# Lingeng56/conformer-pytorch-lightning

Measured on AMD Instinct MI355X. Metric: encoder frames/sec (80-d fbank, T=1000), whole job, higher is better.
Workload: dtype bf16

## Files before the change

conformer-pytorch-lightning_amd/csrc/encoder.cpp:

```cpp
#include <math.h>

#include <stdlib.h>

#include "cfm_common.h"

namespace {

inline const void* eoff(const void* p, int64_t elems, int dt) { return (const char*)p + elems * cfm_elt_size(dt); }

struct Ctx {
    const cfm_layer_io* io;
    int M, D, FF, act_dt, w_dt;
    bool split;
    cfm_stream_t st;
};

int gemm(const Ctx& c, const void* A, int a_dt, int64_t lda, const void* W, const void* Wlo, const float* bias, void* C, int c_dt,
         int64_t ldc, int M, int N, int K, int act, const float* res, float alpha, const uint8_t* row_mask) {
    cfm_gemm_desc d = {};
    d.A = A; d.W = W; d.W_lo = c.split ? Wlo : nullptr; d.bias = bias; d.residual = res; d.row_mask = row_mask; d.C = C;
    d.lda = lda; d.ldc = ldc; d.ldr = ldc; d.M = M; d.N = N; d.K = K;
    d.a_dtype = a_dt; d.w_dtype = c.w_dt; d.c_dtype = c_dt; d.act = act; d.alpha = alpha;
    if (c.split && !Wlo) return cfm_fail(CFM_ERR_ARG, "encoder layer: split mode needs the *_lo weight planes");
    return cfm_gemm(&d, c.st);
// ... 65 lines not shown
    auto after_tail = [&]() -> int {
        if (!io->after_out) return CFM_OK;
        return cfm_layernorm(x_out, io->after_g, io->after_b, io->after_out, CFM_F32, nullptr, nullptr, nullptr, 0, nullptr, eps, M, D, stream);
    };
    CFM_CHECK_ARG(!io->macaron_done || chains, "encoder layer: macaron_done needs the chain path");
    bool ring_written = false;
    static const int ffsplit_rows = getenv("CFM_FFSPLIT_MAX_ROWS") ? atoi(getenv("CFM_FFSPLIT_MAX_ROWS")) : CFM_FFSPLIT_MAX_ROWS;
    const bool ffsplit = chains && s->psum && M <= ffsplit_rows && cfm_ffn_split_supported(D, FF) && s->psum_splits >= FF / 256 &&
                         !io->macaron_done && !io->next_w && w->pw2_w && io->ktaps == 15;
    auto split_desc = [&](int mode) {
        cfm_ffn_split_desc f = {};
        f.M = M; f.D = D; f.mode = mode; f.w_dtype = c.w_dt; f.eps = eps;
        return f;
    };
    const bool pair = chains && s->psum && s->psum_splits >= 3 && M <= CFM_PAIR_MAX_ROWS && cfm_rowchain_pair_supported(D, FF) && !io->macaron_done && !io->next_w;
    if (pair) {
        cfm_rowchain_desc m = {};
        m.x = x_in; m.ln_g = w->ln_ffm_g; m.ln_b = w->ln_ffm_b; m.w1f = w->ffm_w1f; m.w2n = w->ffm_w2n; m.b1 = w->ffm_b1; m.b2 = w->ffm_b2;
        m.psum_out = s->psum; m.M = M; m.D = D; m.FF = FF; m.w_dtype = c.w_dt; m.alpha = 0.5f; m.eps = eps;
        CFM_TRY(cfm_rowchain(&m, stream));
        cfm_rowchain_desc q = {};
        q.x = x_in; q.psum_in = s->psum; q.psum_b2 = w->ffm_b2; q.psum_alpha = 0.5f; q.out_f32 = x_out; q.ln_g = w->ln_mha_g; q.ln_b = w->ln_mha_b;
        q.tail_w = w->qkv_wf; q.tail_b = w->qkv_b; q.tail_out = s->qkv; q.tail_N = 3 * D; q.M = M; q.D = D; q.FF = FF; q.w_dtype = c.w_dt; q.alpha = 1.0f; q.eps = eps;
        q.tail_pair = 1;
        CFM_TRY(cfm_rowchain(&q, stream));
    } else if (ffsplit) {
        cfm_ffn_split_desc f = split_desc(2);
        f.x = x_in; f.ln_g = w->ln_ffm_g; f.ln_b = w->ln_ffm_b; f.w1 = w->ffm_w1f; f.b1 = w->ffm_b1; f.N1 = FF; f.act = CFM_ACT_SILU; f.w2 = w->ffm_w2n;
        f.psum_out = s->psum;
        CFM_TRY(cfm_ffn_split(&f, stream));
        cfm_ffn_split_desc q = split_desc(1);
        q.x = x_in; q.psum = s->psum; q.psum_b2 = w->ffm_b2; q.psum_splits = FF / 256; q.psum_alpha = 0.5f; q.rows_out = x_out;
        q.ln_g = w->ln_mha_g; q.ln_b = w->ln_mha_b; q.w1 = w->qkv_wf; q.b1 = w->qkv_b; q.N1 = 3 * D; q.act = CFM_ACT_NONE; q.out16 = s->qkv; q.ldo = 3 * D;
        ring_written = ring && dk % 4 == 0;
        if (ring_written) { q.kv_ring = io->kv_ring; q.ring_offsets = io->stream_offset; q.ring_T = io->ring_T; q.ring_H = H; q.ring_Tq = io->T; }
        CFM_TRY(cfm_ffn_split(&q, stream));
    } else if (chains && !io->macaron_done && !pair) {
        cfm_rowchain_desc m = {};
        m.x = x_in; m.ln_g = w->ln_ffm_g; m.ln_b = w->ln_ffm_b; m.w1f = w->ffm_w1f; m.w2n = w->ffm_w2n; m.b1 = w->ffm_b1; m.b2 = w->ffm_b2;
        m.ln2_g = w->ln_mha_g; m.ln2_b = w->ln_mha_b; m.out_f32 = x_out; m.tail_w = w->qkv_wf; m.tail_b = w->qkv_b; m.tail_out = s->qkv;
        m.M = M; m.D = D; m.FF = FF; m.tail_N = 3 * D; m.tail_glu = 0; m.w_dtype = c.w_dt; m.alpha = 0.5f; m.eps = eps;
        CFM_TRY(cfm_rowchain(&m, stream));
    }
    const bool fused_ffn = !chains && !c.split && w->ffm_w1f && w->ffm_w2f && w->ff_w1f && w->ff_w2f && (D == 144 || D == 256) &&
                           FF % 32 == 0 && FF <= 2048;

    if (chains) {
    } else if (fused_ffn) {
        CFM_TRY(ffn_fused(c, x_in, w->ln_ffm_g, w->ln_ffm_b, w->ffm_w1f, w->ffm_w2f, w->ffm_b1, w->ffm_b2, nullptr, nullptr,
                          w->ln_mha_g, w->ln_mha_b, x_out, s->xn));
    } else {
        if (!xn_ready) CFM_TRY(cfm_layernorm(x_in, w->ln_ffm_g, w->ln_ffm_b, nullptr, 0, nullptr, nullptr, s->xn, adt, nullptr, eps, M, D, stream));
        CFM_TRY(gemm(c, s->xn, adt, D, w->ffm_w1, w->ffm_w1_lo, w->ffm_b1, s->hid, adt, FF, M, FF, D, CFM_ACT_SILU, nullptr, 0.f, nullptr));
        CFM_TRY(gemm(c, s->hid, adt, FF, w->ffm_w2, w->ffm_w2_lo, w->ffm_b2, x_out, CFM_F32, D, M, D, FF, CFM_ACT_NONE, x_in, 0.5f, nullptr));
        CFM_TRY(cfm_layernorm(x_out, w->ln_mha_g, w->ln_mha_b, nullptr, 0, nullptr, nullptr, s->xn, adt, nullptr, eps, M, D, stream));
// ... 24 lines not shown
        a.k_sb = a.v_sb = sb; a.k_sh = a.v_sh = dk; a.k_st = a.v_st = stt;
    }
    if (has_pos) {
        const int64_t pld = io->pos_proj ? io->pos_proj_ld : D;
        a.p = io->pos_proj ? io->pos_proj : s->pos; a.p_dtype = adt; a.p_sb = io->pos_shared ? 0 : (int64_t)P * pld; a.p_st = P == 1 ? 0 : pld;
        a.bias_u = w->bias_u; a.bias_v = w->bias_v;
    }
    a.mask = io->attn_mask; a.m_sb = io->am_sb; a.m_sq = io->am_sq;
    a.out = s->ctx; a.out_dtype = adt;
    a.B = io->B; a.H = H; a.Tq = io->T; a.Tk = Tk; a.dk = dk;
    a.mma_dtype = c.w_dt; a.split = c.split ? 1 : 0;
    a.scale = 1.0f / sqrtf((float)dk);
    CFM_TRY(cfm_attention(&a, stream));
    if (chains) {
        cfm_rowchain_desc ci = {};
        ci.head_a = s->ctx; ci.head_w = w->out_wf; ci.head_b = w->out_b; ci.head_res = x_out; ci.ln_g = w->ln_conv_g; ci.ln_b = w->ln_conv_b;
        ci.ln_mask = io->pad_valid; ci.out_f32 = x_out; ci.tail_w = w->pw1_wf; ci.tail_b = w->pw1_b; ci.tail_out = s->glu;
        ci.M = M; ci.D = D; ci.FF = FF; ci.tail_N = 2 * D; ci.tail_glu = 1; ci.w_dtype = c.w_dt; ci.alpha = 1.0f; ci.eps = eps;
        if (pair) { ci.tail_pair = 1; ci.out_f32 = s->psum + (int64_t)2 * M * D; }
        const bool cin = cin_merge_flag() != 0 && !pair && !ffsplit && io->next_w && io->next_x_out && D == 256 && FF == 2048 && io->ktaps == 15 && !io->causal_conv &&
                         !io->after_out;
        if (!cin) CFM_TRY(cfm_rowchain(&ci, stream));
        const bool dw_fused = io->ktaps == 15 && !io->causal_conv && cfm_rowchain_dw_supported(D);
        const bool pair_dw = pair && io->ktaps == 15 && !io->causal_conv;
        if (io->causal_conv) {
            CFM_TRY(cfm_dwconv_causal_bn_silu(s->glu, adt, io->conv_cache, w->dw_w, w->dw_b, w->bn_scale, w->bn_shift, s->dw, adt, io->B, io->T, D, io->ktaps, stream));
            if (io->conv_cache) CFM_TRY(cfm_conv_cache_update(s->glu, adt, io->conv_cache, io->B, io->T, D, io->ktaps, stream));
        } else if (!dw_fused && !pair_dw)
            CFM_TRY(cfm_dwconv_bn_silu(s->glu, adt, w->dw_w, w->dw_b, w->bn_scale, w->bn_shift, s->dw, adt, io->B, io->T, D, io->ktaps, stream));
        if (ffsplit) {
            if (dw_fused) {
                cfm_rowchain_desc dh = {};
                dh.head_a = s->glu; dh.head_w = w->pw2_wf; dh.head_b = w->pw2_b; dh.head_res = x_out; dh.head_mask = io->pad_valid;
                dh.dw_w = w->dw_w; dh.dw_b = w->dw_b; dh.dw_scale = w->bn_scale; dh.dw_shift = w->bn_shift; dh.dw_T = io->T; dh.dw_K = 15;
                dh.out_f32 = x_out; dh.M = M; dh.D = D; dh.FF = FF; dh.w_dtype = c.w_dt; dh.alpha = 1.0f; dh.eps = eps;
                CFM_TRY(cfm_rowchain(&dh, stream));
// ... 36 lines not shown
        fi.head_a = dw_fused ? s->glu : s->dw; fi.head_w = w->pw2_wf;
        if (dw_fused) { fi.dw_w = w->dw_w; fi.dw_b = w->dw_b; fi.dw_scale = w->bn_scale; fi.dw_shift = w->bn_shift; fi.dw_T = io->T; fi.dw_K = 15; } fi.head_b = w->pw2_b; fi.head_res = x_out; fi.head_mask = io->pad_valid;
        fi.ln_g = w->ln_ff_g; fi.ln_b = w->ln_ff_b; fi.w1f = w->ff_w1f; fi.w2n = w->ff_w2n; fi.b1 = w->ff_b1; fi.b2 = w->ff_b2;
        fi.ln1_g = w->ln_final_g; fi.ln1_b = w->ln_final_b; fi.out_f32 = x_out;
        if (io->after_out) { fi.ln2_g = io->after_g; fi.ln2_b = io->after_b; fi.out2_f32 = io->after_out; }
        fi.M = M; fi.D = D; fi.FF = FF; fi.w_dtype = c.w_dt; fi.alpha = 0.5f; fi.eps = eps;
        if (io->next_w) {
            const cfm_layer_weights* nw = io->next_w;
            CFM_CHECK_ARG(dw_fused && !io->after_out && io->next_x_out && io->next_x_out != x_out && nw->ffm_w1f && nw->ffm_w2n && nw->qkv_wf && D == 256 && FF == 2048,
                          "encoder layer: chaining into the next block needs the fused depthwise stage, no after_out, a distinct next_x_out and the next "
                          "block's fragment-major packs (D = 256, FF = 2048)");
            fi.out_f32 = nullptr;
            fi.s2_ln_g = nw->ln_ffm_g; fi.s2_ln_b = nw->ln_ffm_b; fi.s2_w1f = nw->ffm_w1f; fi.s2_w2n = nw->ffm_w2n; fi.s2_b1 = nw->ffm_b1; fi.s2_b2 = nw->ffm_b2;
            fi.s2_out_f32 = io->next_x_out; fi.s2_alpha = 0.5f;
            fi.ln2_g = nw->ln_mha_g; fi.ln2_b = nw->ln_mha_b; fi.tail_w = nw->qkv_wf; fi.tail_b = nw->qkv_b; fi.tail_out = s->qkv; fi.tail_N = 3 * D; fi.tail_glu = 0;
            if (cin) {
                fi.cin_a = s->ctx; fi.cin_w = w->out_wf; fi.cin_b = w->out_b; fi.cin_res = x_out; fi.cin_out = io->next_x_out; fi.cin_ln_g = w->ln_conv_g;
                fi.cin_ln_b = w->ln_conv_b; fi.cin_mask = io->pad_valid; fi.cin_tail_w = w->pw1_wf; fi.cin_tail_b = w->pw1_b; fi.head_res = io->next_x_out;
            }
        }
        return cfm_rowchain(&fi, stream);
    }
    CFM_TRY(gemm(c, s->ctx, adt, D, w->out_w, w->out_w_lo, w->out_b, x_out, CFM_F32, D, M, D, D, CFM_ACT_NONE, x_out, 1.0f, nullptr));

    CFM_TRY(cfm_layernorm(x_out, w->ln_conv_g, w->ln_conv_b, nullptr, 0, nullptr, nullptr, s->xn, adt, io->pad_valid, eps, M, D, stream));
    CFM_TRY(gemm(c, s->xn, adt, D, w->pw1_w, w->pw1_w_lo, w->pw1_b, s->glu, adt, D, M, 2 * D, D, CFM_ACT_GLU, nullptr, 0.f, nullptr));
    if (io->causal_conv) {
        CFM_TRY(cfm_dwconv_causal_bn_silu(s->glu, adt, io->conv_cache, w->dw_w, w->dw_b, w->bn_scale, w->bn_shift, s->dw, adt, io->B, io->T, D, io->ktaps, stream));
        if (io->conv_cache) CFM_TRY(cfm_conv_cache_update(s->glu, adt, io->conv_cache, io->B, io->T, D, io->ktaps, stream));
    } else
        CFM_TRY(cfm_dwconv_bn_silu(s->glu, adt, w->dw_w, w->dw_b, w->bn_scale, w->bn_shift, s->dw, adt, io->B, io->T, D, io->ktaps, stream));
    CFM_TRY(gemm(c, s->dw, adt, D, w->pw2_w, w->pw2_w_lo, w->pw2_b, x_out, CFM_F32, D, M, D, D, CFM_ACT_NONE, x_out, 1.0f, io->pad_valid));

    if (fused_ffn) {
// ... 15 lines not shown
```

conformer-pytorch-lightning_amd/csrc/rowchain.hip:

```cpp
#include <stdlib.h>
#include <string>
#include <type_traits>

#include "cfm_common.h"

struct ChainArgs {
    const float* x;
    const u16* head_a;
    const u16* head_w;
    const float* head_b;
    const float* head_res;
    const uint8_t* head_mask;
    const float *dw_w, *dw_b, *dw_scale, *dw_shift;
    int dw_T;
    const float *ln_g, *ln_b;
    const uint8_t* ln_mask;
    const u16 *w1f, *w2n;
    const float *b1, *b2;
    const float *ln1_g, *ln1_b, *ln2_g, *ln2_b;
    float* out_f32;
    void* out16;
    float* out2_f32;
    const u16* tail_w;
    const float* tail_b;
// ... 10 lines not shown
    float* psum_out;
    const float *psum_in, *psum_b2;
    float psum_alpha;
    const u16* cin_a;
    const u16* cin_w;
    const float* cin_b;
    const float* cin_res;
    float* cin_out;
    const float *cin_ln_g, *cin_ln_b;
    const uint8_t* cin_mask;
    const u16* cin_tw;
    const float* cin_tb;
};

#ifdef CFM_CHAIN_STAMPS
__device__ long long cfm_chain_stamps[1024 * 16];
#define CFM_STAMP(i) do { if (threadIdx.x == 0 && blockIdx.x < 1024) { cfm_chain_stamps[blockIdx.x * 16 + (i)] = clock64(); \
        if ((i) == 0 || (i) == 7) cfm_chain_stamps[blockIdx.x * 16 + 8 + ((i) == 7)] = wall_clock64(); } } while (0)
#else
#define CFM_STAMP(i) do { } while (0)
#endif

namespace {

constexpr int RBM = 32;
constexpr int NW = 16;
constexpr int NT = 64 * NW;
constexpr int RPW = RBM / NW;
constexpr int MF = RBM / 16;

template <typename HT, int KS, int NFR, int STRIDE, int MFX = MF>
__device__ __forceinline__ void linear_step(const u16* tile, const u32x4* wp, bool refill, const int (&nx)[NFR], u32x4 (&wr)[NFR * KS],
                                            f32x4 (&acc)[MFX][NFR], int g, int l15) {
// ... 230 lines not shown
#pragma unroll
            for (int i = 0; i < NHALO; ++i) {
                const int id = tid + i * NT;
                const int idc = id < DWROWS * C8 ? id : DWROWS * C8 - 1;
                const int64_t grow = row0 - DWH + idc / C8;
                const int64_t gc = grow < 0 ? 0 : (grow < Mlim ? grow : Mlim - 1);
                const u32x4 v = *(const u32x4*)(a.head_a + gc * D + (idc % C8) * 8);
                hv[i] = (id < DWROWS * C8 && grow >= 0 && grow < Mlim) ? v : (u32x4){0u, 0u, 0u, 0u};
            }
            }
            const int cp = tid < CP * RG ? tid % CP : 0;
            float* const taps = (float*)(lds_a + TAPS_OFF);
            constexpr int NTAP4 = (DWK * D / 4 + NT - 1) / NT;
            static_assert((DWK * D) % 4 == 0, "16-byte pieces of the taps");
            f32x4 tv[NTAP4];
#pragma unroll
            for (int i = 0; i < NTAP4; ++i) tv[i] = *(const f32x4*)(a.dw_w + 4 * (tid + i * NT < DWK * D / 4 ? tid + i * NT : 0));
            const f32x2 pb = *(const f32x2*)(a.dw_b + 2 * cp), ps = *(const f32x2*)(a.dw_scale + 2 * cp), ph = *(const f32x2*)(a.dw_shift + 2 * cp);
            if constexpr (CIN) {
                constexpr int MF3 = CIN_ROWS / 16, RPW3 = CIN_ROWS / NW;
                static_assert(NF2 == NW && RPW3 * NW == CIN_ROWS, "one out-proj fragment and one GLU fragment pair per wavefront, three rows per wavefront");
                const u32x4* cwp = (const u32x4*)a.cin_w + lane;
                u32x4 cwr[KS1];
#pragma unroll
                for (int kk = 0; kk < KS1; ++kk) cwr[kk] = cwp[((int64_t)wave * KS1 + kk) * 64];
                constexpr int NCTX = (CIN_ROWS * CPRW + NT - 1) / NT;
                u32x4 cxv[NCTX];
#pragma unroll
                for (int i = 0; i < NCTX; ++i) {
                    const int id = tid + i * NT < CIN_ROWS * CPRW ? tid + i * NT : CIN_ROWS * CPRW - 1;
                    int64_t grow = row0 - DWH + id / CPRW;
                    grow = grow < 0 ? 0 : (grow < Mlim ? grow : Mlim - 1);
                    cxv[i] = *(const u32x4*)(a.cin_a + grow * D + (id % CPRW) * 8);
                }
                const int ccol = wave * 16 + 4 * g;
                const f32x4 cbb = *(const f32x4*)(a.cin_b + ccol);
                f32x4 crs[MF3];
#pragma unroll
                for (int mf = 0; mf < MF3; ++mf) {
                    int64_t gr = row0 - DWH + mf * 16 + l15;
                    gr = gr < 0 ? 0 : (gr < Mlim ? gr : Mlim - 1);
                    crs[mf] = *(const f32x4*)(a.cin_res + gr * D + ccol);
                }
#pragma unroll
                for (int i = 0; i < NCTX; ++i) {
                    const int id = tid + i * NT;
                    if (id < CIN_ROWS * CPRW) *(u32x4*)(xn + (id / CPRW) * XN_STRIDE + (id % CPRW) * 8) = cxv[i];
                }
#pragma unroll
                for (int i = 0; i < NTAP4; ++i)
                    if (tid + i * NT < DWK * D / 4) *(f32x4*)(taps + 4 * (tid + i * NT)) = tv[i];
                __syncthreads();
                f32x4 cg[VPL], cb[VPL];
#pragma unroll
                for (int it = 0; it < VPL; ++it) {
                    const int c = (lane + 64 * it) * 4;
                    cg[it] = c < D ? *(const f32x4*)(a.cin_ln_g + c) : zero4;
                    cb[it] = c < D ? *(const f32x4*)(a.cin_ln_b + c) : zero4;
                }
                unsigned ckb[RPW3];
#pragma unroll
                for (int rr = 0; rr < RPW3; ++rr) {
                    int64_t gr = row0 - DWH + wave * RPW3 + rr;
                    gr = gr < 0 ? 0 : (gr < Mlim ? gr : Mlim - 1);
                    ckb[rr] = 1u;
                    if (a.cin_mask) ckb[rr] = a.cin_mask[gr];
                }
                {
                    f32x4 cacc[MF3][1];
                    const int nx0[1] = {0};
                    linear_step<HT, KS1, 1, XN_STRIDE, MF3>(xn, cwp, false, nx0, cwr, cacc, g, l15);
#pragma unroll
                    for (int mf = 0; mf < MF3; ++mf) {
                        f32x4 v = cacc[mf][0] + cbb;
                        v += crs[mf];
                        *(f32x4*)(xs + (mf * 16 + l15) * XS_STRIDE + ccol) = v;
                    }
                }
                CFM_STAMP(14);
                const u32x4* ctp = (const u32x4*)a.cin_tw + lane;
                constexpr int CRG = 8;
                u32x4 ctw[CRG];
                auto ct_ptr = [&](int pos) { return ctp + ((int64_t)(2 * wave + pos % 2) * KS1 + pos / 2) * 64; };
#pragma unroll
                for (int t = 0; t < CRG; ++t) ctw[t] = *ct_ptr(t);
                __syncthreads();
                {
                    f32x4 cv[RPW3][VPL];
#pragma unroll
                    for (int rr = 0; rr < RPW3; ++rr) {
                        const int r = wave * RPW3 + rr;
                        const int64_t gr = row0 - DWH + r;
#pragma unroll
                        for (int it = 0; it < VPL; ++it) {
                            const int c = (lane + 64 * it) * 4;
                            cv[rr][it] = c < D ? *(const f32x4*)(xs + r * XS_STRIDE + c) : zero4;
                            if (c < D && r >= DWH && r < DWH + RBM && gr < Mlim) *(f32x4*)(a.cin_out + gr * D + c) = cv[rr][it];
                        }
                    }
                    rows_layernorm<RPW3, VPL, D>(cv, cg, cb, a.eps, lane);
#pragma unroll
                    for (int rr = 0; rr < RPW3; ++rr)
#pragma unroll
                        for (int it = 0; it < VPL; ++it) {
                            const int c = (lane + 64 * it) * 4;
                            if (c < KP) {
                                const f32x4 o = (c < D && ckb[rr] != 0u) ? cv[rr][it] : zero4;
                                *(u32x2*)(xn + (wave * RPW3 + rr) * XN_STRIDE + c) = (u32x2){pack2<HT>(o.x, o.y), pack2<HT>(o.z, o.w)};
                            }
                        }
                }
                const f32x4 tb0 = *(const f32x4*)(a.cin_tb + (2 * wave) * 16 + 4 * g), tb1 = *(const f32x4*)(a.cin_tb + (2 * wave + 1) * 16 + 4 * g);
                __syncthreads();
                CFM_STAMP(15);
                {
                    f32x4 tacc[MF3][2];
                    ring_step<HT, KS1, 2, CRG, XN_STRIDE, decltype(ct_ptr), MF3>(xn, 0, 2 * KS1, ct_ptr, ctw, tacc, g, l15);
#pragma unroll
                    for (int mf = 0; mf < MF3; ++mf) {
                        const int r = mf * 16 + l15;
                        const int64_t gr = row0 - DWH + r;
                        f32x4 v0 = tacc[mf][0] + tb0;
                        const f32x4 v1 = tacc[mf][1] + tb1;
#pragma unroll
                        for (int q = 0; q < 4; ++q) v0[q] *= sigmoidf_(v1[q]);
                        const bool in = gr >= 0 && gr < Mlim;
                        const u32x2 pk = in ? (u32x2){pack2<HT>(v0.x, v0.y), pack2<HT>(v0.z, v0.w)} : (u32x2){0u, 0u};
                        if (r < DWROWS) *(u32x2*)(halo + r * D + wave * 16 + 4 * g) = pk;
                    }
                }
                ln_requests();
            } else {
#pragma unroll
            for (int i = 0; i < NHALO; ++i) {
                const int id = tid + i * NT;
                if (id < DWROWS * C8) *(u32x4*)(halo + (id / C8) * D + (id % C8) * 8) = hv[i];
            }
#pragma unroll
            for (int i = 0; i < NTAP4; ++i)
                if (tid + i * NT < DWK * D / 4) *(f32x4*)(taps + 4 * (tid + i * NT)) = tv[i];
            }
            if constexpr (KP > D) {
                for (int id = tid; id < RBM * (KP - D) / 2; id += NT) {
                    const int r = id / ((KP - D) / 2), c = D + 2 * (id % ((KP - D) / 2));
                    *(unsigned*)(xn + r * XN_STRIDE + c) = 0u;
                }
            }
            __syncthreads();
#pragma unroll
            for (int pass = 0; pass < NPASS; ++pass) {
            const bool worker = tid + pass * NT < CP * RG;
            const int rg = worker ? (tid + pass * NT) / CP : 0;
            if (worker) {
                f32x2 tw[DWK];
                {
                    f32x2 raw[DWK];
#pragma unroll
                    for (int k = 0; k < DWK; ++k) raw[k] = *(const f32x2*)(taps + 2 * cp * DWK + 2 * k);
#pragma unroll
                    for (int k = 0; k < DWK; ++k) {
                        const int i0 = k, i1 = DWK + k;
                        tw[k] = (f32x2){(i0 & 1) ? raw[i0 >> 1].y : raw[i0 >> 1].x, (i1 & 1) ? raw[i1 >> 1].y : raw[i1 >> 1].x};
                    }
// ... 16 lines not shown
                        for (int k = 0; k < DWK; ++k) {
                            const int tt = ti - DWH + k;
                            const f32x2 xv = (tt >= 0 && tt < a.dw_T) ? win[i + k] : (f32x2){0.f, 0.f};
                            acc = (f32x2){fmaf(tw[k].x, xv.x, acc.x), fmaf(tw[k].y, xv.y, acc.y)};
                        }
                    } else {
#pragma unroll
                        for (int k = 0; k < DWK; ++k) acc = (f32x2){fmaf(tw[k].x, win[i + k].x, acc.x), fmaf(tw[k].y, win[i + k].y, acc.y)};
                    }
                    const f32x2 y = (f32x2){fmaf(acc.x + pb.x, ps.x, ph.x), fmaf(acc.y + pb.y, ps.y, ph.y)};
                    const unsigned o = g0 + i < Mlim ? pack2<HT>(siluf_(y.x), siluf_(y.y)) : 0u;
                    *(unsigned*)(xn + (rg * 4 + i) * XN_STRIDE + 2 * cp) = o;
                }
            }
            }
        } else {
            for (int id = tid; id < RBM * CPRW; id += NT) {
                const int r = id / CPRW, c = id % CPRW;
                int64_t grow = row0 + r;
                grow = grow < Mlim ? grow : Mlim - 1;
                const u32x4 v = c * 8 < D ? *(const u32x4*)(a.head_a + grow * D + c * 8) : (u32x4){0u, 0u, 0u, 0u};
                *(u32x4*)(xn + r * XN_STRIDE + c * 8) = v;
            }
        }
        if constexpr (HDW) {
            if constexpr (WIDE) {
#pragma unroll
                for (int t = 0; t < HRG; ++t) wr[t] = *head_ptr(t);
            } else {
#pragma unroll
// ... 93 lines not shown
#pragma unroll
        for (int t = 0; t < RING; ++t)
            if (t < NPOS) ring[t] = *frag_ptr(t);
    }

    if (SEG2 && sg == 1) {
#pragma unroll
        for (int rr = 0; rr < RPW; ++rr)
#pragma unroll
            for (int it = 0; it < VPL; ++it) xres[rr][it] = vcur[rr][it];
        f32x4 w[RPW][VPL];
#pragma unroll
        for (int rr = 0; rr < RPW; ++rr)
#pragma unroll
            for (int it = 0; it < VPL; ++it) w[rr][it] = xres[rr][it];
        rows_layernorm<RPW, VPL, D>(w, nx_g, nx_b, a.eps, lane);
#pragma unroll
        for (int rr = 0; rr < RPW; ++rr)
#pragma unroll
            for (int it = 0; it < VPL; ++it) {
                const int c = (lane + 64 * it) * 4;
                if (c < KP) {
                    const f32x4 o = c < D ? w[rr][it] : zero4;
                    *(u32x2*)(xn + (wave * RPW + rr) * XN_STRIDE + c) = (u32x2){pack2<HT>(o.x, o.y), pack2<HT>(o.z, o.w)};
                }
            }
    } else {
        int64_t (&grows)[RPW] = ln_rows;
        f32x4 (&gam)[VPL] = ln_gam, (&bet)[VPL] = ln_bet;
        bool (&keep)[RPW] = ln_keep;
        if constexpr (HEAD) {
// ... 9 lines not shown
            if (a.out_f32 && (!TSPLIT || tsel == 0)) {
#pragma unroll
                for (int rr = 0; rr < RPW; ++rr)
#pragma unroll
                    for (int it = 0; it < VPL; ++it) {
                        const int c = (lane + 64 * it) * 4;
                        if (c < D && row0 + wave * RPW + rr < Mlim) *(f32x4*)(a.out_f32 + (row0 + wave * RPW + rr) * D + c) = xres[rr][it];
                    }
            }
        }
        f32x4 w[RPW][VPL];
#pragma unroll
        for (int rr = 0; rr < RPW; ++rr)
#pragma unroll
            for (int it = 0; it < VPL; ++it) w[rr][it] = xres[rr][it];
        if (a.ln_g) rows_layernorm<RPW, VPL, D>(w, gam, bet, a.eps, lane);
        if constexpr (WIDE && !MID && !TAIL) {
            if (a.out2_f32) {
#pragma unroll
                for (int rr = 0; rr < RPW; ++rr)
#pragma unroll
                    for (int it = 0; it < VPL; ++it) {
                        const int c = (lane + 64 * it) * 4;
                        if (c < D && row0 + wave * RPW + rr < Mlim) *(f32x4*)(a.out2_f32 + (row0 + wave * RPW + rr) * D + c) = w[rr][it];
                    }
            }
        }
#pragma unroll
        for (int rr = 0; rr < RPW; ++rr)
#pragma unroll
            for (int it = 0; it < VPL; ++it) {
// ... 309 lines not shown
    CFM_CHECK_ARG(!head || (d->head_w && d->head_b && d->head_res), "cfm_rowchain: head needs weights, bias and residual");
    CFM_CHECK_ARG(!mid || (d->w2n && d->b1 && d->b2 && d->FF > 0), "cfm_rowchain: the feed-forward needs w1f, w2n, b1, b2 and FF");
    CFM_CHECK_ARG(!tail || (d->tail_b && d->tail_out && d->tail_N % 16 == 0 && d->tail_N > 0 && (!d->tail_glu || d->tail_N % 32 == 0)),
                  "cfm_rowchain: tail needs bias, output and N %% 16 == 0 (GLU: N %% 32 == 0)");
    CFM_CHECK_ARG(!tail || (mid ? d->ln2_g != nullptr : true), "cfm_rowchain: a tail after the FFN takes its input from the second LayerNorm");
    const bool ps_out = d->psum_out != nullptr, ps_in = d->psum_in != nullptr;
    CFM_CHECK_ARG(!ps_out || (mid && !head && !tail && !seg2 && !d->ln1_g && !d->ln2_g && cfm_rowchain_pair_supported(d->D, d->FF)),
                  "cfm_rowchain: psum_out needs a feed-forward chain at D = 512 without head / tail / post norms");
    CFM_CHECK_ARG(!ps_in || (!head && !mid && d->D == 512 && d->psum_b2 && d->x), "cfm_rowchain: psum_in needs a rows chain (no head, no feed-forward) at D = 512, x and psum_b2");
    CFM_CHECK_ARG(!d->tail_pair || (!mid && d->D == 512 && (tail ? (d->tail_N / 16) % 2 == 0 : (head && dw && d->out_f32 && !d->ln_g)) && (!head || d->out_f32 != d->head_res)),
                  "cfm_rowchain: tail_pair needs a chain without a feed-forward at D = 512 -- with a tail, or the depthwise head alone (no LayerNorm, rows to out_f32) -- "
                  "and (with a head) out_f32 distinct from head_res");
    ChainArgs a;
    a.psum_out = d->psum_out; a.psum_in = d->psum_in; a.psum_b2 = d->psum_b2; a.psum_alpha = d->psum_alpha;
    const bool cin = d->cin_a != nullptr;
    CFM_CHECK_ARG(!cin || (seg2 && dw && d->D == 256 && d->cin_w && d->cin_b && d->cin_res && d->cin_out && d->cin_ln_g && d->cin_ln_b && d->cin_tail_w && d->cin_tail_b &&
                           d->head_res == d->cin_out && d->cin_out != d->cin_res),
                  "cfm_rowchain: the conv-in input stage (cin_*) needs the depthwise + final + next-macaron chain at D = 256, all of its operands, head_res == cin_out "
                  "and cin_out distinct from cin_res (halo rows of cin_res belong to other tiles)");
    a.cin_a = (const u16*)d->cin_a; a.cin_w = (const u16*)d->cin_w; a.cin_b = d->cin_b; a.cin_res = d->cin_res; a.cin_out = d->cin_out; a.cin_ln_g = d->cin_ln_g;
    a.cin_ln_b = d->cin_ln_b; a.cin_mask = d->cin_mask; a.cin_tw = (const u16*)d->cin_tail_w; a.cin_tb = d->cin_tail_b;
    a.x = d->x; a.head_a = (const u16*)d->head_a; a.head_w = (const u16*)d->head_w; a.head_b = d->head_b; a.head_res = d->head_res;
    a.dw_w = d->dw_w; a.dw_b = d->dw_b; a.dw_scale = d->dw_scale; a.dw_shift = d->dw_shift; a.dw_T = d->dw_T;
    a.head_mask = d->head_mask; a.ln_g = d->ln_g; a.ln_b = d->ln_b; a.ln_mask = d->ln_mask; a.w1f = (const u16*)d->w1f; a.w2n = (const u16*)d->w2n;
    a.b1 = d->b1; a.b2 = d->b2; a.ln1_g = d->ln1_g; a.ln1_b = d->ln1_b; a.ln2_g = d->ln2_g; a.ln2_b = d->ln2_b; a.out_f32 = d->out_f32;
    a.out16 = d->out16; a.out2_f32 = d->out2_f32; a.tail_w = (const u16*)d->tail_w; a.tail_b = d->tail_b; a.tail_out = d->tail_out; a.M = d->M;
    a.tail_N = d->tail_N; a.out16_dtype = d->w_dtype; a.alpha = d->alpha; a.eps = d->eps;
    a.s2_ln_g = d->s2_ln_g; a.s2_ln_b = d->s2_ln_b; a.s2_w1f = (const u16*)d->s2_w1f; a.s2_w2n = (const u16*)d->s2_w2n; a.s2_b1 = d->s2_b1;
    a.s2_b2 = d->s2_b2; a.s2_out_f32 = d->s2_out_f32; a.s2_alpha = d->s2_alpha;
    hipStream_t s = (hipStream_t)stream;
    const bool bf = d->w_dtype == CFM_BF16;
    const int tfrags = tail ? d->tail_N / 16 : 0;
    const int tsteps = !tail ? 0 : d->tail_glu ? (tfrags / 2 + NW - 1) / NW : (tfrags + NW - 1) / NW;
    const double M = (double)d->M;
    const double fl_head = head ? 2.0 * M * d->D * d->D : 0.0, fl_mid = mid ? 4.0 * M * d->D * d->FF : 0.0,
                 fl_tail = tail ? 2.0 * M * d->D * d->tail_N : 0.0;
    const double fl = fl_head + fl_mid * (seg2 ? 2.0 : 1.0) + fl_tail + (dw ? 2.0 * M * d->D * 15 : 0.0);
#define CFM_RC(HT, DD, FFV, HS, MIDV, TS, GLU, NAME) return launch_chain<HT, DD, FFV, HS, false, MIDV, TS, GLU>(a, s, NAME, fl)
#define CFM_RCDW(HT, DD, FFV, NAME) return launch_chain<HT, DD, FFV, 1, true, true, 0, false>(a, s, NAME, fl)
    if (d->D == 256 && (!mid || d->FF == 2048)) {
        if (cin && seg2 && head && dw && tail && !d->tail_glu && tsteps == 3) { if (bf) return launch_chain<BF16, 256, 2048, 1, true, true, 3, false, true, false, false, true>(a, s, "chain_convin_dwfinal_macaron_bf16_d256", fl + 2.0 * M * d->D * 3 * d->D); else return launch_chain<F16, 256, 2048, 1, true, true, 3, false, true, false, false, true>(a, s, "chain_convin_dwfinal_macaron_f16_d256", fl + 2.0 * M * d->D * 3 * d->D); }
        if (seg2 && head && dw && tail && !d->tail_glu && tsteps == 3) { if (bf) return launch_chain<BF16, 256, 2048, 1, true, true, 3, false, true>(a, s, "chain_dwfinal_macaron_bf16_d256", fl); else return launch_chain<F16, 256, 2048, 1, true, true, 3, false, true>(a, s, "chain_dwfinal_macaron_f16_d256", fl); }
        if (seg2) return cfm_fail(CFM_ERR_UNSUPPORTED, "cfm_rowchain: a second segment only on the depthwise + final chain followed by a QKV tail (D = 256)");
        if (!head && mid && tail && !d->tail_glu && tsteps == 3) { if (bf) CFM_RC(BF16, 256, 2048, 0, true, 3, false, "chain_macaron_bf16_d256"); else CFM_RC(F16, 256, 2048, 0, true, 3, false, "chain_macaron_f16_d256"); }
        if (head && !mid && tail && d->tail_glu && tsteps == 1) { if (bf) CFM_RC(BF16, 256, 64, 1, false, 1, true, "chain_convin_bf16_d256"); else CFM_RC(F16, 256, 64, 1, false, 1, true, "chain_convin_f16_d256"); }
        if (head && mid && !tail && dw) { if (bf) CFM_RCDW(BF16, 256, 2048, "chain_dwfinal_bf16_d256"); else CFM_RCDW(F16, 256, 2048, "chain_dwfinal_f16_d256"); }
        if (head && !mid && !tail && dw) { if (bf) return launch_chain<BF16, 256, 64, 1, true, false, 0, false>(a, s, "chain_dwhead_bf16_d256", fl); else return launch_chain<F16, 256, 64, 1, true, false, 0, false>(a, s, "chain_dwhead_f16_d256", fl); }
        if (head && mid && !tail) { if (bf) CFM_RC(BF16, 256, 2048, 1, true, 0, false, "chain_final_bf16_d256"); else CFM_RC(F16, 256, 2048, 1, true, 0, false, "chain_final_f16_d256"); }
        if (!head && !mid && tail && !d->tail_glu && tsteps == 3) { if (bf) CFM_RC(BF16, 256, 64, 0, false, 3, false, "chain_qkv_bf16_d256"); else CFM_RC(F16, 256, 64, 0, false, 3, false, "chain_qkv_f16_d256"); }
        if (!head && !mid && !tail) { if (bf) CFM_RC(BF16, 256, 64, 0, false, 0, false, "chain_rows_bf16_d256"); else CFM_RC(F16, 256, 64, 0, false, 0, false, "chain_rows_f16_d256"); }
    } else if (d->D == 144 && (!mid || d->FF == 576)) {
        if (!head && mid && tail && !d->tail_glu && tsteps == 2) { if (bf) CFM_RC(BF16, 144, 576, 0, true, 2, false, "chain_macaron_bf16_d144"); else CFM_RC(F16, 144, 576, 0, true, 2, false, "chain_macaron_f16_d144"); }
        if (head && !mid && tail && d->tail_glu && tsteps == 1) { if (bf) CFM_RC(BF16, 144, 64, 1, false, 1, true, "chain_convin_bf16_d144"); else CFM_RC(F16, 144, 64, 1, false, 1, true, "chain_convin_f16_d144"); }
        if (head && mid && !tail && dw) { if (bf) CFM_RCDW(BF16, 144, 576, "chain_dwfinal_bf16_d144"); else CFM_RCDW(F16, 144, 576, "chain_dwfinal_f16_d144"); }
        if (head && mid && !tail) { if (bf) CFM_RC(BF16, 144, 576, 1, true, 0, false, "chain_final_bf16_d144"); else CFM_RC(F16, 144, 576, 1, true, 0, false, "chain_final_f16_d144"); }
        if (!head && !mid && tail && !d->tail_glu && tsteps == 2) { if (bf) CFM_RC(BF16, 144, 64, 0, false, 2, false, "chain_qkv_bf16_d144"); else CFM_RC(F16, 144, 64, 0, false, 2, false, "chain_qkv_f16_d144"); }
// ... 19 lines not shown
```

conformer-pytorch-lightning_amd/encoder.py:

```python
import torch
import torch.nn as nn

import cfm
from attention import PositionalEncoding, RelativePositionalEncoding
from convolution import ConvolutionSubSampling
from encoder_layer import ConformerEncoderLayer
from utils import make_attn_mask, make_pad_mask

_NO_MASK = torch.ones((0, 0, 0))


class ConformerEncoder(nn.Module):

    def __init__(self, input_dim, kernel_size, encoder_dim, dropout, attention_dropout, pos_enc_dropout, hidden_dim,
                 num_heads, encoder_num_layers, cmvn=None, max_len=5000, use_relative=False, use_dynamic_chunk_size=False,
                 use_dynamic_left_chunk=False, static_chunk_size=-1):
        super().__init__()
        pe_cls = RelativePositionalEncoding if use_relative else PositionalEncoding
        self.position_encoding = pe_cls(encoder_dim, pos_enc_dropout, max_len)
        self.embed = ConvolutionSubSampling(input_dim=input_dim, output_dim=encoder_dim, pos_enc=self.position_encoding)
        self.encoders = nn.ModuleList([
            ConformerEncoderLayer(encoder_dim, kernel_size, dropout, attention_dropout, hidden_dim, num_heads, use_relative)
            for _ in range(encoder_num_layers)])
        self.encoder_dim = encoder_dim
# ... 16 lines not shown
        y_after = torch.empty_like(x) if fuse_after else None
        import encoder_layer as _el
        e0 = self.encoders[0]
        chain = (_el.CHAIN_BLOCKS and fuse_after and caches is None and conv is None and self.encoder_dim == 256 and
                 e0.hidden_dim == 2048 and e0.kernel_size == 15 and not getattr(e0.conv_module, "causal", False) and
                 all(b.chain_ready(prec) for b in self.encoders) and
                 not (streaming and _el.SPLIT_FFN_FEW_ROWS and _el.split_rows(x.size(0) * x.size(1), self.encoder_dim, e0.hidden_dim)))
        for i, block in enumerate(self.encoders):
            nxt = self.encoders[i + 1].norm_ff_macaron if i + 1 < n else None
            cache_i = None
            if caches is not None and caches.dim() == 5 and caches.size(0) > 0:
                cache_i = caches[i]
            elif caches is not None and caches.dim() == 4 and caches.size(0) > 0:
                cache_i = caches[i:i + 1]
            pp = None if proj is None else (proj[:, i * self.encoder_dim:], proj.stride(0))
            out, nc = block.fused_forward(cur, attn_mask, pos_embed, pad_mask, cache_i, xn_ready=ready, next_norm=nxt,
                                          out=bufs[i & 1], want_cache=caches is not None, pos_proj=pp, pos_shared=pos_shared,
                                          ring=None if ring is None else (ring[0][i], ring[1]), conv_cache=None if conv is None else conv[i],
                                          chain_next=(self.encoders[i + 1], bufs[(i + 1) & 1]) if chain and i + 1 < n else None,
                                          macaron_done=chain and i > 0, split_ffn=streaming,
                                          after=(self.after_norm.weight.detach(), self.after_norm.bias.detach(), y_after)
                                          if fuse_after and i + 1 == n else None)
            if new_caches is not None:
                new_caches.append(nc[:, :, keep_from:, :])
            cur, ready = out, nxt is not None
        if fuse_after:
            return y_after, new_caches
        y, _ = cfm.layernorm(cur.view(-1, cur.size(-1)), self.after_norm.weight.detach(), self.after_norm.bias.detach(),
                             eps=self.after_norm.eps)
        return y.view_as(cur), new_caches

    def _cmvn_args(self, inputs):
        m = self.global_cmvn
        if m is None:
            return inputs, None
# ... 341 lines not shown
```

conformer-pytorch-lightning_amd/encoder_layer.py:

```python
import ctypes

import torch
import torch.nn as nn

import cfm
from cfm import packing
from attention import MultiHeadSelfAttentionModule, RelativeMultiHeadSelfAttentionModule, _mask_args
from convolution import ConvolutionModule
from feedforward import PositionwiseFeedForwardModule, _inference_only

_ABSENT = torch.ones((0, 0, 0), dtype=torch.bool)
PAIR_MAX_ROWS = 4096
SPLIT_FFN_FEW_ROWS = True


import os as _os
_SPLIT_MAX_ROWS = int(_os.environ.get("CFM_FFSPLIT_MAX_ROWS", "1536"))


def split_rows(M, D, FF):
    return M <= _SPLIT_MAX_ROWS and D == 256 and FF % 256 == 0 and FF > 0


CHAIN_BLOCKS = True
# ... 115 lines not shown
            io.causal_conv = 1
            if conv_cache is not None:
                if conv_cache.dtype != torch.float32 or tuple(conv_cache.shape) != (B, self.kernel_size - 1, D) or not conv_cache.is_contiguous():
                    raise RuntimeError("conv_cache must be contiguous float32 (B, kernel_size-1, D)")
                cfm.require_hip(conv_cache)
                io.conv_cache = conv_cache.data_ptr()
        elif conv_cache is not None:
            raise RuntimeError("a conv cache needs the opt-in causal convolution (conv_module.causal = True)")
        if out is None:
            out = torch.empty_like(x)
        if chain_next is not None:
            nxt_w = chain_next[0]._weights(prec)
            if chain_next[1].data_ptr() == out.data_ptr() or chain_next[1].shape != out.shape or chain_next[1].dtype != torch.float32:
                raise RuntimeError("chain_next: the next block's output buffer must be a distinct float32 tensor of the same shape")
            io.next_w, io.next_x_out = ctypes.cast(ctypes.pointer(nxt_w), ctypes.c_void_p), chain_next[1].data_ptr()
        io.macaron_done = 1 if macaron_done else 0
        ng = nb = None
        if next_norm is not None:
            ng, nb = next_norm.weight.data_ptr(), next_norm.bias.data_ptr()
        cfm.check(cfm.lib().cfm_encoder_layer_forward(ctypes.byref(w), ctypes.byref(s), ctypes.byref(io), x.data_ptr(),
                                                      out.data_ptr(), 1 if xn_ready else 0, ng, nb, cfm.stream()),
                  "cfm_encoder_layer_forward")
        return out, new_cache

    def train_forward(self, inputs, inputs_attn_mask, inputs_pad_mask):
        from cfm import autograd as ag
        cfm.require_hip(inputs)
        B, T, D = inputs.shape
        m8, m_str = _mask_args(inputs_attn_mask, B, T, T)
        keep = None
        if inputs_pad_mask is not None and inputs_pad_mask.dim() >= 3 and inputs_pad_mask.size(2) > 0:
# ... 21 lines not shown
```

Measured before the change: 26.66 million.

## Fuse conv-in stage into last block's depthwise+final chain

Extends the conv-in merge (attention out-projection, residual, conv LayerNorm and pointwise-GLU) so it also runs for the last encoder block, fused into the depthwise + final chain kernel instead of a separate rowchain launch. A new macaron_done=2 mode and a reworked buffer assignment let the last block read its residual from a distinct buffer, because halo rows must not be overwritten. The kernel now adds the residual per row after the out-proj instead of per fragment, and issues the depthwise-tap loads later to shorten register live ranges. Extra timing stamps are added, but they are compiled only under a debug macro.

```diff
diff --git a/conformer-pytorch-lightning_amd/csrc/encoder.cpp b/conformer-pytorch-lightning_amd/csrc/encoder.cpp
--- a/conformer-pytorch-lightning_amd/csrc/encoder.cpp
+++ b/conformer-pytorch-lightning_amd/csrc/encoder.cpp
@@ -103,6 +103,12 @@
         return f;
     };
     const bool pair = chains && s->psum && s->psum_splits >= 3 && M <= CFM_PAIR_MAX_ROWS && cfm_rowchain_pair_supported(D, FF) && !io->macaron_done && !io->next_w;
+    CFM_CHECK_ARG(io->macaron_done == 0 || io->macaron_done == 1 || (io->macaron_done == 2 && !io->next_w), "encoder layer: macaron_done is 0, 1 or (without next_w) 2");
+    const bool cin_shape = chains && cin_merge_flag() != 0 && !pair && !ffsplit && D == 256 && FF == 2048 && io->ktaps == 15 && !io->causal_conv;
+    const bool cin_next = cin_shape && io->next_w && io->next_x_out && !io->after_out;
+    const bool cin_last = cin_shape && !io->next_w && (io->macaron_done == 2 || (io->macaron_done == 0 && s->hid && (int64_t)FF * cfm_elt_size(adt) >= (int64_t)D * 4));
+    float* const slab = (float*)s->hid;
+    const float* const xr = io->macaron_done == 2 ? x_in : (cin_last ? slab : x_out);
     if (pair) {
         cfm_rowchain_desc m = {};
         m.x = x_in; m.ln_g = w->ln_ffm_g; m.ln_b = w->ln_ffm_b; m.w1f = w->ffm_w1f; m.w2n = w->ffm_w2n; m.b1 = w->ffm_b1; m.b2 = w->ffm_b2;
@@ -127,7 +133,7 @@
     } else if (chains && !io->macaron_done && !pair) {
         cfm_rowchain_desc m = {};
         m.x = x_in; m.ln_g = w->ln_ffm_g; m.ln_b = w->ln_ffm_b; m.w1f = w->ffm_w1f; m.w2n = w->ffm_w2n; m.b1 = w->ffm_b1; m.b2 = w->ffm_b2;
-        m.ln2_g = w->ln_mha_g; m.ln2_b = w->ln_mha_b; m.out_f32 = x_out; m.tail_w = w->qkv_wf; m.tail_b = w->qkv_b; m.tail_out = s->qkv;
+        m.ln2_g = w->ln_mha_g; m.ln2_b = w->ln_mha_b; m.out_f32 = cin_last ? slab : x_out; m.tail_w = w->qkv_wf; m.tail_b = w->qkv_b; m.tail_out = s->qkv;
         m.M = M; m.D = D; m.FF = FF; m.tail_N = 3 * D; m.tail_glu = 0; m.w_dtype = c.w_dt; m.alpha = 0.5f; m.eps = eps;
         CFM_TRY(cfm_rowchain(&m, stream));
     }
@@ -182,12 +188,11 @@
     CFM_TRY(cfm_attention(&a, stream));
     if (chains) {
         cfm_rowchain_desc ci = {};
-        ci.head_a = s->ctx; ci.head_w = w->out_wf; ci.head_b = w->out_b; ci.head_res = x_out; ci.ln_g = w->ln_conv_g; ci.ln_b = w->ln_conv_b;
+        ci.head_a = s->ctx; ci.head_w = w->out_wf; ci.head_b = w->out_b; ci.head_res = xr; ci.ln_g = w->ln_conv_g; ci.ln_b = w->ln_conv_b;
         ci.ln_mask = io->pad_valid; ci.out_f32 = x_out; ci.tail_w = w->pw1_wf; ci.tail_b = w->pw1_b; ci.tail_out = s->glu;
         ci.M = M; ci.D = D; ci.FF = FF; ci.tail_N = 2 * D; ci.tail_glu = 1; ci.w_dtype = c.w_dt; ci.alpha = 1.0f; ci.eps = eps;
         if (pair) { ci.tail_pair = 1; ci.out_f32 = s->psum + (int64_t)2 * M * D; }
-        const bool cin = cin_merge_flag() != 0 && !pair && !ffsplit && io->next_w && io->next_x_out && D == 256 && FF == 2048 && io->ktaps == 15 && !io->causal_conv &&
-                         !io->after_out;
+        const bool cin = cin_next || cin_last;
         if (!cin) CFM_TRY(cfm_rowchain(&ci, stream));
         const bool dw_fused = io->ktaps == 15 && !io->causal_conv && cfm_rowchain_dw_supported(D);
         const bool pair_dw = pair && io->ktaps == 15 && !io->causal_conv;
@@ -254,10 +259,14 @@
             fi.s2_ln_g = nw->ln_ffm_g; fi.s2_ln_b = nw->ln_ffm_b; fi.s2_w1f = nw->ffm_w1f; fi.s2_w2n = nw->ffm_w2n; fi.s2_b1 = nw->ffm_b1; fi.s2_b2 = nw->ffm_b2;
             fi.s2_out_f32 = io->next_x_out; fi.s2_alpha = 0.5f;
             fi.ln2_g = nw->ln_mha_g; fi.ln2_b = nw->ln_mha_b; fi.tail_w = nw->qkv_wf; fi.tail_b = nw->qkv_b; fi.tail_out = s->qkv; fi.tail_N = 3 * D; fi.tail_glu = 0;
-            if (cin) {
+            if (cin_next) {
                 fi.cin_a = s->ctx; fi.cin_w = w->out_wf; fi.cin_b = w->out_b; fi.cin_res = x_out; fi.cin_out = io->next_x_out; fi.cin_ln_g = w->ln_conv_g;
                 fi.cin_ln_b = w->ln_conv_b; fi.cin_mask = io->pad_valid; fi.cin_tail_w = w->pw1_wf; fi.cin_tail_b = w->pw1_b; fi.head_res = io->next_x_out;
             }
+        }
+        if (cin_last) {
+            fi.cin_a = s->ctx; fi.cin_w = w->out_wf; fi.cin_b = w->out_b; fi.cin_res = xr; fi.cin_out = x_out; fi.cin_ln_g = w->ln_conv_g;
+            fi.cin_ln_b = w->ln_conv_b; fi.cin_mask = io->pad_valid; fi.cin_tail_w = w->pw1_wf; fi.cin_tail_b = w->pw1_b; fi.head_res = x_out;
         }
         return cfm_rowchain(&fi, stream);
     }
diff --git a/conformer-pytorch-lightning_amd/csrc/rowchain.hip b/conformer-pytorch-lightning_amd/csrc/rowchain.hip
--- a/conformer-pytorch-lightning_amd/csrc/rowchain.hip
+++ b/conformer-pytorch-lightning_amd/csrc/rowchain.hip
@@ -48,9 +48,10 @@
 };
 
 #ifdef CFM_CHAIN_STAMPS
-__device__ long long cfm_chain_stamps[1024 * 16];
-#define CFM_STAMP(i) do { if (threadIdx.x == 0 && blockIdx.x < 1024) { cfm_chain_stamps[blockIdx.x * 16 + (i)] = clock64(); \
-        if ((i) == 0 || (i) == 7) cfm_chain_stamps[blockIdx.x * 16 + 8 + ((i) == 7)] = wall_clock64(); } } while (0)
+#define CFM_NSTAMP 32
+__device__ long long cfm_chain_stamps[1024 * CFM_NSTAMP];
+#define CFM_STAMP(i) do { if (threadIdx.x == 0 && blockIdx.x < 1024) { cfm_chain_stamps[blockIdx.x * CFM_NSTAMP + (i)] = clock64(); \
+        if ((i) == 0 || (i) == 7) cfm_chain_stamps[blockIdx.x * CFM_NSTAMP + 8 + ((i) == 7)] = wall_clock64(); } } while (0)
 #else
 #define CFM_STAMP(i) do { } while (0)
 #endif
@@ -311,9 +312,13 @@
             constexpr int NTAP4 = (DWK * D / 4 + NT - 1) / NT;
             static_assert((DWK * D) % 4 == 0, "16-byte pieces of the taps");
             f32x4 tv[NTAP4];
-#pragma unroll
-            for (int i = 0; i < NTAP4; ++i) tv[i] = *(const f32x4*)(a.dw_w + 4 * (tid + i * NT < DWK * D / 4 ? tid + i * NT : 0));
-            const f32x2 pb = *(const f32x2*)(a.dw_b + 2 * cp), ps = *(const f32x2*)(a.dw_scale + 2 * cp), ph = *(const f32x2*)(a.dw_shift + 2 * cp);
+            f32x2 pb, ps, ph;
+            auto dw_requests = [&]() {
+#pragma unroll
+                for (int i = 0; i < NTAP4; ++i) tv[i] = *(const f32x4*)(a.dw_w + 4 * (tid + i * NT < DWK * D / 4 ? tid + i * NT : 0));
+                pb = *(const f32x2*)(a.dw_b + 2 * cp); ps = *(const f32x2*)(a.dw_scale + 2 * cp); ph = *(const f32x2*)(a.dw_shift + 2 * cp);
+            };
+            if constexpr (!CIN) dw_requests();
             if constexpr (CIN) {
                 constexpr int MF3 = CIN_ROWS / 16, RPW3 = CIN_ROWS / NW;
                 static_assert(NF2 == NW && RPW3 * NW == CIN_ROWS, "one out-proj fragment and one GLU fragment pair per wavefront, three rows per wavefront");
@@ -332,22 +337,25 @@
                 }
                 const int ccol = wave * 16 + 4 * g;
                 const f32x4 cbb = *(const f32x4*)(a.cin_b + ccol);
-                f32x4 crs[MF3];
-#pragma unroll
-                for (int mf = 0; mf < MF3; ++mf) {
-                    int64_t gr = row0 - DWH + mf * 16 + l15;
+                f32x4 crs[RPW3][VPL];
+#pragma unroll
+                for (int rr = 0; rr < RPW3; ++rr) {
+                    int64_t gr = row0 - DWH + wave * RPW3 + rr;
                     gr = gr < 0 ? 0 : (gr < Mlim ? gr : Mlim - 1);
-                    crs[mf] = *(const f32x4*)(a.cin_res + gr * D + ccol);
-                }
+#pragma unroll
+                    for (int it = 0; it < VPL; ++it) {
+                        const int c = (lane + 64 * it) * 4;
+                        crs[rr][it] = c < D ? *(const f32x4*)(a.cin_res + gr * D + c) : zero4;
+                    }
+                }
+                CFM_STAMP(16);
 #pragma unroll
                 for (int i = 0; i < NCTX; ++i) {
                     const int id = tid + i * NT;
                     if (id < CIN_ROWS * CPRW) *(u32x4*)(xn + (id / CPRW) * XN_STRIDE + (id % CPRW) * 8) = cxv[i];
                 }
-#pragma unroll
-                for (int i = 0; i < NTAP4; ++i)
-                    if (tid + i * NT < DWK * D / 4) *(f32x4*)(taps + 4 * (tid + i * NT)) = tv[i];
                 __syncthreads();
+                CFM_STAMP(17);
                 f32x4 cg[VPL], cb[VPL];
 #pragma unroll
                 for (int it = 0; it < VPL; ++it) {
@@ -367,10 +375,10 @@
                     f32x4 cacc[MF3][1];
                     const int nx0[1] = {0};
                     linear_step<HT, KS1, 1, XN_STRIDE, MF3>(xn, cwp, false, nx0, cwr, cacc, g, l15);
+                    CFM_STAMP(18);
 #pragma unroll
                     for (int mf = 0; mf < MF3; ++mf) {
-                        f32x4 v = cacc[mf][0] + cbb;
-                        v += crs[mf];
+                        const f32x4 v = cacc[mf][0] + cbb;
                         *(f32x4*)(xs + (mf * 16 + l15) * XS_STRIDE + ccol) = v;
                     }
                 }
@@ -391,11 +399,12 @@
 #pragma unroll
                         for (int it = 0; it < VPL; ++it) {
                             const int c = (lane + 64 * it) * 4;
-                            cv[rr][it] = c < D ? *(const f32x4*)(xs + r * XS_STRIDE + c) : zero4;
+                            cv[rr][it] = c < D ? *(const f32x4*)(xs + r * XS_STRIDE + c) + crs[rr][it] : zero4;
                             if (c < D && r >= DWH && r < DWH + RBM && gr < Mlim) *(f32x4*)(a.cin_out + gr * D + c) = cv[rr][it];
                         }
                     }
                     rows_layernorm<RPW3, VPL, D>(cv, cg, cb, a.eps, lane);
+                    CFM_STAMP(19);
 #pragma unroll
                     for (int rr = 0; rr < RPW3; ++rr)
 #pragma unroll
@@ -407,12 +416,14 @@
                             }
                         }
                 }
+                dw_requests();
                 const f32x4 tb0 = *(const f32x4*)(a.cin_tb + (2 * wave) * 16 + 4 * g), tb1 = *(const f32x4*)(a.cin_tb + (2 * wave + 1) * 16 + 4 * g);
                 __syncthreads();
                 CFM_STAMP(15);
                 {
                     f32x4 tacc[MF3][2];
                     ring_step<HT, KS1, 2, CRG, XN_STRIDE, decltype(ct_ptr), MF3>(xn, 0, 2 * KS1, ct_ptr, ctw, tacc, g, l15);
+                    CFM_STAMP(20);
 #pragma unroll
                     for (int mf = 0; mf < MF3; ++mf) {
                         const int r = mf * 16 + l15;
@@ -426,6 +437,9 @@
                         if (r < DWROWS) *(u32x2*)(halo + r * D + wave * 16 + 4 * g) = pk;
                     }
                 }
+#pragma unroll
+                for (int i = 0; i < NTAP4; ++i)
+                    if (tid + i * NT < DWK * D / 4) *(f32x4*)(taps + 4 * (tid + i * NT)) = tv[i];
                 ln_requests();
             } else {
 #pragma unroll
@@ -444,6 +458,7 @@
                 }
             }
             __syncthreads();
+            CFM_STAMP(21);
 #pragma unroll
             for (int pass = 0; pass < NPASS; ++pass) {
             const bool worker = tid + pass * NT < CP * RG;
@@ -490,6 +505,7 @@
                 }
             }
             }
+            CFM_STAMP(22);
         } else {
             for (int id = tid; id < RBM * CPRW; id += NT) {
                 const int r = id / CPRW, c = id % CPRW;
@@ -613,7 +629,9 @@
         for (int rr = 0; rr < RPW; ++rr)
 #pragma unroll
             for (int it = 0; it < VPL; ++it) w[rr][it] = xres[rr][it];
+        CFM_STAMP(25);
         rows_layernorm<RPW, VPL, D>(w, nx_g, nx_b, a.eps, lane);
+        CFM_STAMP(26);
 #pragma unroll
         for (int rr = 0; rr < RPW; ++rr)
 #pragma unroll
@@ -653,7 +671,9 @@
         for (int rr = 0; rr < RPW; ++rr)
 #pragma unroll
             for (int it = 0; it < VPL; ++it) w[rr][it] = xres[rr][it];
+        CFM_STAMP(23);
         if (a.ln_g) rows_layernorm<RPW, VPL, D>(w, gam, bet, a.eps, lane);
+        CFM_STAMP(24);
         if constexpr (WIDE && !MID && !TAIL) {
             if (a.out2_f32) {
 #pragma unroll
@@ -993,9 +1013,9 @@
     ChainArgs a;
     a.psum_out = d->psum_out; a.psum_in = d->psum_in; a.psum_b2 = d->psum_b2; a.psum_alpha = d->psum_alpha;
     const bool cin = d->cin_a != nullptr;
-    CFM_CHECK_ARG(!cin || (seg2 && dw && d->D == 256 && d->cin_w && d->cin_b && d->cin_res && d->cin_out && d->cin_ln_g && d->cin_ln_b && d->cin_tail_w && d->cin_tail_b &&
+    CFM_CHECK_ARG(!cin || ((seg2 || (mid && !tail)) && dw && d->D == 256 && d->cin_w && d->cin_b && d->cin_res && d->cin_out && d->cin_ln_g && d->cin_ln_b && d->cin_tail_w && d->cin_tail_b &&
                            d->head_res == d->cin_out && d->cin_out != d->cin_res),
-                  "cfm_rowchain: the conv-in input stage (cin_*) needs the depthwise + final + next-macaron chain at D = 256, all of its operands, head_res == cin_out "
+                  "cfm_rowchain: the conv-in input stage (cin_*) needs the depthwise + final (+ next-macaron) chain at D = 256, all of its operands, head_res == cin_out "
                   "and cin_out distinct from cin_res (halo rows of cin_res belong to other tiles)");
     a.cin_a = (const u16*)d->cin_a; a.cin_w = (const u16*)d->cin_w; a.cin_b = d->cin_b; a.cin_res = d->cin_res; a.cin_out = d->cin_out; a.cin_ln_g = d->cin_ln_g;
     a.cin_ln_b = d->cin_ln_b; a.cin_mask = d->cin_mask; a.cin_tw = (const u16*)d->cin_tail_w; a.cin_tb = d->cin_tail_b;
@@ -1019,6 +1039,8 @@
 #define CFM_RCDW(HT, DD, FFV, NAME) return launch_chain<HT, DD, FFV, 1, true, true, 0, false>(a, s, NAME, fl)
     if (d->D == 256 && (!mid || d->FF == 2048)) {
         if (cin && seg2 && head && dw && tail && !d->tail_glu && tsteps == 3) { if (bf) return launch_chain<BF16, 256, 2048, 1, true, true, 3, false, true, false, false, true>(a, s, "chain_convin_dwfinal_macaron_bf16_d256", fl + 2.0 * M * d->D * 3 * d->D); else return launch_chain<F16, 256, 2048, 1, true, true, 3, false, true, false, false, true>(a, s, "chain_convin_dwfinal_macaron_f16_d256", fl + 2.0 * M * d->D * 3 * d->D); }
+        if (cin && !seg2 && head && dw && mid && !tail) { if (bf) return launch_chain<BF16, 256, 2048, 1, true, true, 0, false, false, false, false, true>(a, s, "chain_convin_dwfinal_last_bf16_d256", fl + 2.0 * M * d->D * 3 * d->D); else return launch_chain<F16, 256, 2048, 1, true, true, 0, false, false, false, false, true>(a, s, "chain_convin_dwfinal_last_f16_d256", fl + 2.0 * M * d->D * 3 * d->D); }
+        if (cin) return cfm_fail(CFM_ERR_UNSUPPORTED, "cfm_rowchain: the conv-in input stage only in front of the depthwise + final chain, alone or followed by the next block's macaron chain (D = 256, FF = 2048)");
         if (seg2 && head && dw && tail && !d->tail_glu && tsteps == 3) { if (bf) return launch_chain<BF16, 256, 2048, 1, true, true, 3, false, true>(a, s, "chain_dwfinal_macaron_bf16_d256", fl); else return launch_chain<F16, 256, 2048, 1, true, true, 3, false, true>(a, s, "chain_dwfinal_macaron_f16_d256", fl); }
         if (seg2) return cfm_fail(CFM_ERR_UNSUPPORTED, "cfm_rowchain: a second segment only on the depthwise + final chain followed by a QKV tail (D = 256)");
         if (!head && mid && tail && !d->tail_glu && tsteps == 3) { if (bf) CFM_RC(BF16, 256, 2048, 0, true, 3, false, "chain_macaron_bf16_d256"); else CFM_RC(F16, 256, 2048, 0, true, 3, false, "chain_macaron_f16_d256"); }
diff --git a/conformer-pytorch-lightning_amd/encoder.py b/conformer-pytorch-lightning_amd/encoder.py
--- a/conformer-pytorch-lightning_amd/encoder.py
+++ b/conformer-pytorch-lightning_amd/encoder.py
@@ -54,11 +54,12 @@
             elif caches is not None and caches.dim() == 4 and caches.size(0) > 0:
                 cache_i = caches[i:i + 1]
             pp = None if proj is None else (proj[:, i * self.encoder_dim:], proj.stride(0))
-            out, nc = block.fused_forward(cur, attn_mask, pos_embed, pad_mask, cache_i, xn_ready=ready, next_norm=nxt,
-                                          out=bufs[i & 1], want_cache=caches is not None, pos_proj=pp, pos_shared=pos_shared,
+            last_chained = chain and i > 0 and i + 1 == n
+            out, nc = block.fused_forward(bufs[i & 1] if last_chained else cur, attn_mask, pos_embed, pad_mask, cache_i, xn_ready=ready, next_norm=nxt,
+                                          out=bufs[(i + 1) & 1] if last_chained else bufs[i & 1], want_cache=caches is not None, pos_proj=pp, pos_shared=pos_shared,
                                           ring=None if ring is None else (ring[0][i], ring[1]), conv_cache=None if conv is None else conv[i],
                                           chain_next=(self.encoders[i + 1], bufs[(i + 1) & 1]) if chain and i + 1 < n else None,
-                                          macaron_done=chain and i > 0, split_ffn=streaming,
+                                          macaron_done=2 if last_chained else (chain and i > 0), split_ffn=streaming,
                                           after=(self.after_norm.weight.detach(), self.after_norm.bias.detach(), y_after)
                                           if fuse_after and i + 1 == n else None)
             if new_caches is not None:
diff --git a/conformer-pytorch-lightning_amd/encoder_layer.py b/conformer-pytorch-lightning_amd/encoder_layer.py
--- a/conformer-pytorch-lightning_amd/encoder_layer.py
+++ b/conformer-pytorch-lightning_amd/encoder_layer.py
@@ -153,7 +153,7 @@
             if chain_next[1].data_ptr() == out.data_ptr() or chain_next[1].shape != out.shape or chain_next[1].dtype != torch.float32:
                 raise RuntimeError("chain_next: the next block's output buffer must be a distinct float32 tensor of the same shape")
             io.next_w, io.next_x_out = ctypes.cast(ctypes.pointer(nxt_w), ctypes.c_void_p), chain_next[1].data_ptr()
-        io.macaron_done = 1 if macaron_done else 0
+        io.macaron_done = int(macaron_done)
         ng = nb = None
         if next_norm is not None:
             ng, nb = next_norm.weight.data_ptr(), next_norm.bias.data_ptr()
```

Result: no change. 26.75 million, median of 6 (+0.4%).
